# IRVLUTD/handnet-pipeline

Hardware: AMD Instinct MI355X
Metric: end-to-end frames/sec (FCOS+A2J, 640x480) (higher is better)
Workload: dtype f16x3 (fp32 values split into fp16 hi+lo, 3 MFMAs, fp32 accumulate; fp32 I/O); 1 GPU; Full HandNet pipeline (FCOS -> crop -> A2J), 640x480 RGB-D (BASELINE config 4); batch_per_gpu=32, global_batch=32, frame=640x480 RGB-D, parallelism=frames sharded over 1 GPU(s), one all-gather of per-frame records per step, rccl_ranks=1, ipc_mode=HSA_ENABLE_IPC_MODE_LEGACY=0, hipgraph=False

## Files before the change

### handnet-pipeline_amd/csrc/conv1x1_stream.hip

```cpp
#include "hn_common.h"

namespace {

typedef float f32x4 __attribute__((ext_vector_type(4)));
typedef _Float16 f16x8 __attribute__((ext_vector_type(8)));
typedef __attribute__((address_space(3))) void lds_void;

constexpr int kTileBytes = 32 * 1024;
constexpr int kStages = 2;
constexpr int kWaves = 8;
constexpr int kThreads = kWaves * 64;

struct StreamParams {
  const _Float16* x;
  const _Float16* w;
  const float* bias;
  const void* res;
  void* y;
  int M, Cout, relu, out_split, res_mode, res_split, res_h, res_w, OH, OW;
  int ys, rs;
  int tiles;
  unsigned x_records;
  unsigned mg_ohow, sh_ohow, mg_ow, sh_ow, mg_oh, sh_oh;
  int* range_flag;
};

__device__ __forceinline__ int fastdiv(int n, unsigned mg, unsigned sh) { return mg ? (int)(__umulhi((unsigned)n, mg) >> sh) : n; }

template <int CB>
__global__ __launch_bounds__(kThreads, 4) void conv1x1_stream_kernel(const StreamParams p) {
  constexpr int kTilePix = kTileBytes / (CB * 128);
  constexpr int PIX_BYTES = CB * 128;
  constexpr int CHUNKS = CB * 8;
  constexpr int TILE_BYTES = kTileBytes;
  constexpr int PASSES = TILE_BYTES / (kThreads * 16);
  static_assert(CB == 2 || CB == 4, "Cin = 64 or 128");
  static_assert(TILE_BYTES % (kThreads * 16) == 0, "a tile is a whole number of DMA passes");
  extern __shared__ __attribute__((aligned(1024))) char smem[];
  const int tid = threadIdx.x, lane = tid & 63, wave = tid >> 6, lg = lane >> 4, px = lane & 15;
  const int n0 = blockIdx.y * 256 + wave * 32;

  f16x8 bh[2][CB], bl[2][CB];
#pragma unroll
  for (int j = 0; j < 2; ++j)
#pragma unroll
    for (int cb = 0; cb < CB; ++cb) {
      const _Float16* q = p.w + ((long)(n0 + j * 16 + px) * CB + cb) * 64 + lg * 8;
      bh[j][cb] = *reinterpret_cast<const f16x8*>(q);
      bl[j][cb] = *reinterpret_cast<const f16x8*>(q + 32);
    }
  const int nsub = (lg & 1) * 16 + (lg >> 1) * 8;
  const int n = n0 + nsub;
  float* bias_lds = reinterpret_cast<float*>(smem + kStages * kTileBytes);
  if (tid < 256) bias_lds[tid] = p.bias ? p.bias[blockIdx.y * 256 + tid] : 0.f;

  const __amdgpu_buffer_rsrc_t rsrc = __builtin_amdgcn_make_buffer_rsrc((void*)p.x, 0, (int)p.x_records, 0x00020000);
  static_assert((kThreads / CHUNKS) % 16 == 0, "a DMA pass covers whole 16-pixel groups");
  const unsigned src_off = (unsigned)((tid / CHUNKS) * PIX_BYTES + (((tid % CHUNKS) ^ ((tid / CHUNKS) & 15)) << 4));
  const int wave_base = __builtin_amdgcn_readfirstlane(wave) * 64 * 16;
  auto dma_tile = [&](int t, int stage) {
#pragma unroll
    for (int ps = 0; ps < PASSES; ++ps)
      __builtin_amdgcn_raw_ptr_buffer_load_lds(rsrc, (lds_void*)(smem + stage * TILE_BYTES + ps * kThreads * 16 + wave_base), 16,
                                               (int)src_off, t * TILE_BYTES + ps * kThreads * 16, 0, 0);
  };
  auto frag = [&](int stage, int pt, int cb, int pl) {
    const int pixel = pt * 16 + px;
    return *reinterpret_cast<const f16x8*>(smem + stage * TILE_BYTES + pixel * PIX_BYTES + (((cb * 8 + pl * 4 + lg) ^ px) << 4));
  };

  const int ohow = p.OH * p.OW;
  const int t0 = blockIdx.x, dt = gridDim.x;
  dma_tile(t0, 0);
  int stage = 0;
  for (int t = t0; t < p.tiles; t += dt) {
    asm volatile("s_waitcnt vmcnt(0)" ::: "memory");
    __syncthreads();
    if (t + dt < p.tiles) dma_tile(t + dt, stage ^ 1);
#pragma unroll
    for (int pt = 0; pt < kTilePix / 16; ++pt) {
      f32x4 acc0 = {0.f, 0.f, 0.f, 0.f}, acc1 = acc0;
#pragma unroll
      for (int c2 = 0; c2 < CB; c2 += 2) {
        f16x8 ah[2], al[2];
#pragma unroll
        for (int c = 0; c < 2; ++c) {
          ah[c] = frag(stage, pt, c2 + c, 0);
          al[c] = frag(stage, pt, c2 + c, 1);
        }
#pragma unroll
        for (int c = 0; c < 2; ++c) {
          const int cb = c2 + c;
          acc0 = __builtin_amdgcn_mfma_f32_16x16x32_f16(bh[0][cb], al[c], acc0, 0, 0, 0);
          acc1 = __builtin_amdgcn_mfma_f32_16x16x32_f16(bh[1][cb], al[c], acc1, 0, 0, 0);
          acc0 = __builtin_amdgcn_mfma_f32_16x16x32_f16(bl[0][cb], ah[c], acc0, 0, 0, 0);
          acc1 = __builtin_amdgcn_mfma_f32_16x16x32_f16(bl[1][cb], ah[c], acc1, 0, 0, 0);
          acc0 = __builtin_amdgcn_mfma_f32_16x16x32_f16(bh[0][cb], ah[c], acc0, 0, 0, 0);
          acc1 = __builtin_amdgcn_mfma_f32_16x16x32_f16(bh[1][cb], ah[c], acc1, 0, 0, 0);
        }
        if (c2 + 2 < CB) __builtin_amdgcn_sched_barrier(0);
      }
#pragma unroll
      for (int r = 0; r < 4; ++r) {
        const auto s = __builtin_amdgcn_permlane16_swap(__float_as_uint(acc0[r]), __float_as_uint(acc1[r]), false, false);
        acc0[r] = __uint_as_float(s[0]);
        acc1[r] = __uint_as_float(s[1]);
      }
      const int m = t * kTilePix + pt * 16 + px;
      if (m >= p.M) continue;
      float v[8];
      const f32x4 bias0 = *reinterpret_cast<const f32x4*>(bias_lds + wave * 32 + nsub);
      const f32x4 bias1 = *reinterpret_cast<const f32x4*>(bias_lds + wave * 32 + nsub + 4);
#pragma unroll
      for (int e = 0; e < 4; ++e) {
        v[e] = acc0[e] + bias0[e];
        v[4 + e] = acc1[e] + bias1[e];
      }
      if (p.res_mode) {
        long rpix = m;
        if (p.res_mode == 2) {
          const int img = fastdiv(m, p.mg_ohow, p.sh_ohow);
          const int rem = m - img * ohow;
          const int oh = fastdiv(rem, p.mg_ow, p.sh_ow), ow = rem - oh * p.OW;
          const int sh_ = fastdiv(oh * p.res_h, p.mg_oh, p.sh_oh), sw_ = fastdiv(ow * p.res_w, p.mg_ow, p.sh_ow);
          rpix = ((long)img * p.res_h + sh_) * p.res_w + sw_;
        }
        if (p.res_split) {
          const _Float16* q16 = reinterpret_cast<const _Float16*>(p.res) + rpix * p.rs + (n >> 5) * 64 + (n & 31);
          const f16x8 rh = *reinterpret_cast<const f16x8*>(q16), rl = *reinterpret_cast<const f16x8*>(q16 + 32);
#pragma unroll
          for (int e = 0; e < 8; ++e) v[e] += (float)rh[e] + (float)rl[e];
        } else {
          const float* q32 = reinterpret_cast<const float*>(p.res) + rpix * p.rs + n;
          const f32x4 r0 = *reinterpret_cast<const f32x4*>(q32), r1 = *reinterpret_cast<const f32x4*>(q32 + 4);
#pragma unroll
          for (int e = 0; e < 4; ++e) {
            v[e] += r0[e];
            v[4 + e] += r1[e];
          }
        }
      }
      if (p.relu) {
#pragma unroll
        for (int e = 0; e < 8; ++e) v[e] = hn::relu(v[e]);
      }
      if (p.out_split) {
        if (p.range_flag) hn::range_note_n<8>(p.range_flag, v);
        f16x8 hi, lo;
#pragma unroll
        for (int e = 0; e < 8; ++e) {
          const _Float16 h = (_Float16)v[e];
          hi[e] = h;
          lo[e] = (_Float16)(v[e] - (float)h);
        }
        _Float16* q16 = reinterpret_cast<_Float16*>(p.y) + (long)m * p.ys + (n >> 5) * 64 + (n & 31);
        *reinterpret_cast<f16x8*>(q16) = hi;
        *reinterpret_cast<f16x8*>(q16 + 32) = lo;
      } else {
        float* q32 = reinterpret_cast<float*>(p.y) + (long)m * p.ys + n;
        *reinterpret_cast<f32x4*>(q32) = f32x4{v[0], v[1], v[2], v[3]};
        *reinterpret_cast<f32x4*>(q32 + 4) = f32x4{v[4], v[5], v[6], v[7]};
      }
    }
    stage ^= 1;
  }
  asm volatile("s_waitcnt vmcnt(0)" ::: "memory");
}

}

namespace hn {

static void magic_u31(unsigned d, unsigned& mg, unsigned& sh) {
  if (d <= 1) { mg = 0; sh = 0; return; }
  unsigned k = 0;
  while ((1ull << k) < d) ++k;
  mg = (unsigned)(((1ull << (31 + k)) + d - 1) / d);
  sh = k - 1;
}

bool conv1x1_stream_applies(const hn_conv_desc* d, bool has_gn, bool has_group) {
  const int64_t m = (int64_t)d->n * d->oh * d->ow;
  return !env_flags().no_stream && !has_gn && !has_group && d->r == 1 && d->s == 1 && d->stride == 1 && d->pad == 0 && d->dil == 1 &&
         (d->cin == 64 || d->cin == 128) && d->cout % 256 == 0 && d->terms != 1 && d->tile == HN_TILE_AUTO &&
         (d->in_pix_stride == 0 || d->in_pix_stride == 2 * d->cin) && (d->relu_cols == 0 || d->relu_cols >= d->cout) &&
         m >= (int64_t)65536 && (int64_t)d->oh * d->res_h < ((int64_t)1 << 31) && (int64_t)d->ow * d->res_w < ((int64_t)1 << 31) && m * d->cin * 4 < ((int64_t)1 << 31) - ((int64_t)64 << 20);
}

bool conv1x1_stream_operands_ok(const hn_conv_desc* d, const void* x16, const void* w16, const float* bias, const void* residual,
                                const void* y) {
  const int ys = d->out_pix_stride ? d->out_pix_stride : (d->out_split ? 2 : 1) * d->cout;
  const int rs = d->res_pix_stride ? d->res_pix_stride : (d->res_split ? 2 : 1) * d->cout;
  return (uintptr_t)x16 % 16 == 0 && (uintptr_t)w16 % 16 == 0 && (uintptr_t)y % 16 == 0 && (!bias || (uintptr_t)bias % 16 == 0) &&
         (!residual || (uintptr_t)residual % 16 == 0) && (d->out_split ? ys % 64 == 0 : ys % 4 == 0) &&
         (d->res_mode == 0 || (d->res_split ? rs % 64 == 0 : rs % 4 == 0));
}

int conv1x1_stream(const hn_conv_desc* d, const void* x16, const void* w16, const float* bias, const void* residual, void* y,
                   hipStream_t st) {
  StreamParams p;
  p.x = (const _Float16*)x16; p.w = (const _Float16*)w16; p.bias = bias; p.res = d->res_mode ? residual : nullptr; p.y = y;
  p.M = d->n * d->oh * d->ow; p.Cout = d->cout; p.relu = d->relu_cols > 0; p.out_split = d->out_split;
  p.res_mode = d->res_mode; p.res_split = d->res_split; p.res_h = d->res_h; p.res_w = d->res_w; p.OH = d->oh; p.OW = d->ow;
  p.ys = d->out_pix_stride ? d->out_pix_stride : (d->out_split ? 2 : 1) * d->cout;
  p.rs = d->res_pix_stride ? d->res_pix_stride : (d->res_split ? 2 : 1) * d->cout;
  const int tile_pix = kTileBytes / (d->cin * 4);
  p.tiles = cdiv(p.M, tile_pix);
  magic_u31((unsigned)(d->oh * d->ow), p.mg_ohow, p.sh_ohow);
  magic_u31((unsigned)d->ow, p.mg_ow, p.sh_ow);
  magic_u31((unsigned)d->oh, p.mg_oh, p.sh_oh);
  p.x_records = (unsigned)((int64_t)p.M * d->cin * 4);
  p.range_flag = range_flag_ptr();
  const int cb = d->cin / 32;
  const int lds = kStages * kTileBytes + 1024;
  int dev = 0, cus = 256;
  HN_CHECK_HIP(hipGetDevice(&dev));
  static int cu_count[64] = {};
  if (dev >= 0 && dev < 64) {
    if (!cu_count[dev]) {
      hipDeviceProp_t prop;
      HN_CHECK_HIP(hipGetDeviceProperties(&prop, dev));
      cu_count[dev] = prop.multiProcessorCount;
    }
    cus = cu_count[dev];
  }
  const int groups = d->cout / 256;
  int gx = cus * 2 / groups;
  gx = gx < 1 ? 1 : (gx > p.tiles ? p.tiles : gx);
  static bool attr_set[2][64] = {};
  auto set_attr = [&](const void* fn, int which) -> int {
    if (dev < 0 || dev >= 64 || !attr_set[which][dev]) {
      HN_CHECK_HIP(hipFuncSetAttribute(fn, hipFuncAttributeMaxDynamicSharedMemorySize, lds));
      if (dev >= 0 && dev < 64) attr_set[which][dev] = true;
    }
    return HN_OK;
  };
  if (cb == 2) {
    const int s = set_attr((const void*)conv1x1_stream_kernel<2>, 0);
    if (s != HN_OK) return s;
    hipLaunchKernelGGL(conv1x1_stream_kernel<2>, dim3(gx, groups), dim3(kThreads), lds, st, p);
  } else {
    const int s = set_attr((const void*)conv1x1_stream_kernel<4>, 1);
    if (s != HN_OK) return s;
    hipLaunchKernelGGL(conv1x1_stream_kernel<4>, dim3(gx, groups), dim3(kThreads), lds, st, p);
  }
  HN_CHECK_LAUNCH("conv1x1_stream_kernel");
  return HN_OK;
}

}
```

### handnet-pipeline_amd/csrc/hn_common.h

```cpp
#pragma once
#include <hip/hip_runtime.h>
#include <stdarg.h>
#include <stdint.h>
#include <stdio.h>

#include "../../include/handnet_hip.h"

namespace hn {

char* err_buf();
int fail(int code, const char* fmt, ...);
int* range_flag_ptr();
struct EnvFlags {
  bool no_rs, no_rs32, split_generic, no_halo, no_thin, thin_tap, thin_flat, no_fuse_last_gn, pre_generic, no_multi,
      halo_stamps, splitk_fill512, no_stream, no_mixed, no_deepk, no_fused_reduce, thin_nogroup;
};
const EnvFlags& env_flags();
struct Tuning {
  double splitk_fix = 1.0, splitk_tk = 1.0, splitk_red0 = 1.0, splitk_plane = 1.0;
};
const Tuning& tuning();
bool conv3x3_halo_applies(const hn_conv_desc* d, bool has_gn, bool has_group, const void* residual);
bool conv3x3_halo_operands_ok(const hn_conv_desc* d, const void* x16, const void* w16, const float* bias, const void* residual,
                              const void* y);
int conv3x3_halo(const hn_conv_desc* d, const void* x16, const void* w16, const float* bias, const void* residual, void* y,
                 hipStream_t st);
int stem_pool_direct(const void* x16, int n, int ph, int pw, const void* w16, const float* bias, void* y, int terms, hipStream_t st);
bool conv1x1_stream_applies(const hn_conv_desc* d, bool has_gn, bool has_group);
bool conv1x1_stream_operands_ok(const hn_conv_desc* d, const void* x16, const void* w16, const float* bias, const void* residual,
                                const void* y);
int conv1x1_stream(const hn_conv_desc* d, const void* x16, const void* w16, const float* bias, const void* residual, void* y,
                   hipStream_t st);

struct CarryHook {
  const void* job;
  bool dry;
};
int launch_conv_carry(const void* conv_params, size_t conv_params_bytes, int grid_x, int groups, int terms, int lds_bytes,
                      const void* job, hipStream_t st);
int conv_grouped_run(const hn_conv_desc* d, const hn_conv_group* group, void* stream, const CarryHook* carry);

int tickets_nonzero_main(int64_t* count);
int tickets_nonzero_multi(int64_t* count);

#define HN_CHECK_ARG(cond, ...)                          \
  do {                                                   \
    if (!(cond)) return hn::fail(HN_ERR_ARG, __VA_ARGS__); \
  } while (0)

#define HN_CHECK_HIP(expr)                                                         \
  do {                                                                             \
    hipError_t e_ = (expr);                                                        \
    if (e_ != hipSuccess)                                                          \
      return hn::fail(HN_ERR_HIP, "%s failed: %s", #expr, hipGetErrorString(e_)); \
  } while (0)

#define HN_CHECK_LAUNCH(name)                                                          \
  do {                                                                                 \
    hipError_t e_ = hipGetLastError();                                                 \
    if (e_ != hipSuccess)                                                              \
      return hn::fail(HN_ERR_HIP, "launch of %s failed: %s", name, hipGetErrorString(e_)); \
  } while (0)

static inline int cdiv(int64_t a, int64_t b) { return (int)((a + b - 1) / b); }

__device__ __forceinline__ void range_note(int* flag, float v) {
  if (!(fabsf(v) <= 65504.f)) *flag = 1;
}
__device__ __forceinline__ float max_nan(float a, float b) { return __builtin_elementwise_maximum(a, b); }
__device__ __forceinline__ float relu(float v) { return max_nan(v, 0.f); }
__device__ __forceinline__ float range_mag(float a, float b) { return max_nan(fabsf(a), fabsf(b)); }
__device__ __forceinline__ bool range_bad(float v) { return !(fabsf(v) <= 65504.f); }
template <int N>
__device__ __forceinline__ void range_note_n(int* flag, const float (&v)[N]) {
  float m = fabsf(v[0]);
#pragma unroll
  for (int e = 1; e < N; ++e) m = max_nan(m, fabsf(v[e]));
  if (!(m <= 65504.f)) *flag = 1;
}
__device__ __forceinline__ void range_note_input(int* flag, float v) {
  if (!(fabsf(v) <= 65504.f)) flag[fabsf(v) <= 3.402823466e38f ? 1 : 2] = 1;
}

}
```

### handnet-pipeline_amd/csrc/hn_common.hip

```cpp
#include "hn_common.h"

#include <stdlib.h>

#include <string.h>

__device__ int g_range_flag[4];
static thread_local int g_range_check_on = 0;
static thread_local int* g_range_bound = nullptr;
struct RangeScope { int on; int* bound; };
static thread_local RangeScope g_range_stack[8];
static thread_local int g_range_depth = 0;

namespace hn {

int* range_flag_ptr() {
  if (!g_range_check_on) return nullptr;
  if (g_range_bound) return g_range_bound;
  static int* ptrs[64] = {nullptr};
  int dev = 0;
  if (hipGetDevice(&dev) != hipSuccess || dev < 0 || dev >= 64) return nullptr;
  if (!ptrs[dev]) {
    void* p = nullptr;
    if (hipGetSymbolAddress(&p, HIP_SYMBOL(g_range_flag)) != hipSuccess) return nullptr;
    ptrs[dev] = (int*)p;
  }
  return ptrs[dev];
}

char* err_buf() {
  static thread_local char buf[512] = {0};
  return buf;
}

int fail(int code, const char* fmt, ...) {
  va_list ap;
  va_start(ap, fmt);
  vsnprintf(err_buf(), 512, fmt, ap);
  va_end(ap);
  return code;
}

}

extern "C" int hn_abi_version(void) { return HN_ABI_VERSION; }

extern "C" int hn_debug_tickets_nonzero(int64_t* count) {
  HN_CHECK_ARG(count, "hn_debug_tickets_nonzero: null pointer");
  *count = 0;
  if (int rc = hn::tickets_nonzero_main(count)) return rc;
  return hn::tickets_nonzero_multi(count);
}

namespace hn {
static EnvFlags g_env = {};
const EnvFlags& env_flags() { return g_env; }
static Tuning g_tuning;
const Tuning& tuning() { return g_tuning; }
}

extern "C" int hn_set_tuning(const char* name, double value) {
  HN_CHECK_ARG(name && value > 0.0, "hn_set_tuning: null name or non-positive value");
  struct Entry { const char* name; double hn::Tuning::*field; };
  static const Entry table[] = {{"splitk_fix", &hn::Tuning::splitk_fix}, {"splitk_tk", &hn::Tuning::splitk_tk},
                                {"splitk_red0", &hn::Tuning::splitk_red0}, {"splitk_plane", &hn::Tuning::splitk_plane}};
  for (const Entry& e : table)
    if (strcmp(e.name, name) == 0) {
      hn::g_tuning.*(e.field) = value;
      return HN_OK;
    }
  return hn::fail(HN_ERR_ARG, "hn_set_tuning: unknown constant '%s'", name);
}

extern "C" int hn_set_form(const char* name, int value) {
  HN_CHECK_ARG(name, "hn_set_form: null name");
  struct Entry { const char* name; bool hn::EnvFlags::*field; };
  static const Entry table[] = {
      {"conv_no_rs", &hn::EnvFlags::no_rs},
      {"conv_no_rs32", &hn::EnvFlags::no_rs32},
      {"split_generic", &hn::EnvFlags::split_generic},
      {"conv_no_halo", &hn::EnvFlags::no_halo},
      {"preprocess_generic", &hn::EnvFlags::pre_generic},
      {"conv_no_multi", &hn::EnvFlags::no_multi},
      {"no_fuse_last_gn", &hn::EnvFlags::no_fuse_last_gn},
      {"no_thin_outputs", &hn::EnvFlags::no_thin},
      {"thin_form_tap", &hn::EnvFlags::thin_tap},
      {"thin_form_flat", &hn::EnvFlags::thin_flat},
      {"thin_no_group", &hn::EnvFlags::thin_nogroup},
      {"halo_stamps", &hn::EnvFlags::halo_stamps},
      {"splitk_fill512", &hn::EnvFlags::splitk_fill512},
      {"conv_no_stream", &hn::EnvFlags::no_stream},
      {"conv_no_mixed", &hn::EnvFlags::no_mixed},
      {"conv_no_deepk", &hn::EnvFlags::no_deepk},
      {"conv_no_fused_reduce", &hn::EnvFlags::no_fused_reduce},
  };
  for (const Entry& e : table)
    if (strcmp(e.name, name) == 0) {
      hn::g_env.*(e.field) = value != 0;
      return HN_OK;
    }
  return hn::fail(HN_ERR_ARG, "hn_set_form: unknown form '%s'", name);
}

extern "C" const char* hn_last_error(void) { return hn::err_buf(); }

extern "C" int hn_device_info(int* cu_count, int* clock_khz, char* arch_name, int arch_name_len) {
  int dev = 0;
  HN_CHECK_HIP(hipGetDevice(&dev));
  hipDeviceProp_t prop;
  HN_CHECK_HIP(hipGetDeviceProperties(&prop, dev));
  if (cu_count) *cu_count = prop.multiProcessorCount;
  if (clock_khz) *clock_khz = prop.clockRate;
  if (arch_name && arch_name_len > 0) {
    strncpy(arch_name, prop.gcnArchName, arch_name_len - 1);
    arch_name[arch_name_len - 1] = 0;
  }
  return HN_OK;
}

extern "C" int hn_device_pci_bus_id(char* out, int out_len) {
  HN_CHECK_ARG(out && out_len >= 16, "hn_device_pci_bus_id: buffer of at least 16 bytes");
  int dev = 0;
  HN_CHECK_HIP(hipGetDevice(&dev));
  HN_CHECK_HIP(hipDeviceGetPCIBusId(out, out_len, dev));
  return HN_OK;
}

extern "C" int hn_event_create(void** ev) {
  HN_CHECK_ARG(ev, "hn_event_create: null");
  hipEvent_t e;
  HN_CHECK_HIP(hipEventCreate(&e));
  *ev = (void*)e;
  return HN_OK;
}

extern "C" int hn_event_destroy(void* ev) {
  HN_CHECK_HIP(hipEventDestroy((hipEvent_t)ev));
  return HN_OK;
}

extern "C" int hn_event_record(void* ev, void* stream) {
  HN_CHECK_HIP(hipEventRecord((hipEvent_t)ev, (hipStream_t)stream));
  return HN_OK;
}

extern "C" int hn_event_elapsed_ms(void* start, void* stop, float* ms) {
  HN_CHECK_ARG(ms, "hn_event_elapsed_ms: null");
  HN_CHECK_HIP(hipEventSynchronize((hipEvent_t)stop));
  HN_CHECK_HIP(hipEventElapsedTime(ms, (hipEvent_t)start, (hipEvent_t)stop));
  return HN_OK;
}

extern "C" int hn_range_check_enable(int on) {
  g_range_check_on = on ? 1 : 0;
  return HN_OK;
}

extern "C" int hn_range_check_enabled(void) { return g_range_check_on; }

extern "C" int hn_range_check_bind(int32_t* block) {
  g_range_bound = block;
  return HN_OK;
}

extern "C" int hn_range_scope_begin(int32_t* block, int on) {
  HN_CHECK_ARG(g_range_depth < 8, "hn_range_scope_begin: more than 8 nested scopes on this thread");
  g_range_stack[g_range_depth++] = RangeScope{g_range_check_on, g_range_bound};
  g_range_check_on = on ? 1 : 0;
  g_range_bound = on ? block : nullptr;
  return HN_OK;
}

extern "C" int hn_range_scope_end(void) {
  HN_CHECK_ARG(g_range_depth > 0, "hn_range_scope_end: no open scope on this thread");
  const RangeScope s = g_range_stack[--g_range_depth];
  g_range_check_on = s.on;
  g_range_bound = s.bound;
  return HN_OK;
}

extern "C" int hn_range_check_fetch(int* flag, int reset, void* stream) {
  HN_CHECK_ARG(flag, "hn_range_check_fetch: null");
  void* p = nullptr;
  int words[4] = {0, 0, 0, 0};
  HN_CHECK_HIP(hipGetSymbolAddress(&p, HIP_SYMBOL(g_range_flag)));
  HN_CHECK_HIP(hipMemcpyAsync(words, p, sizeof(words), hipMemcpyDeviceToHost, (hipStream_t)stream));
  HN_CHECK_HIP(hipStreamSynchronize((hipStream_t)stream));
  *flag = (words[0] ? HN_RANGE_ACTIVATION : 0) | (words[1] ? HN_RANGE_INPUT : 0) | (words[2] ? HN_RANGE_INPUT_NONFINITE : 0);
  if (reset) {
    HN_CHECK_HIP(hipMemsetAsync(p, 0, sizeof(words), (hipStream_t)stream));
    HN_CHECK_HIP(hipStreamSynchronize((hipStream_t)stream));
  }
  return HN_OK;
}

namespace {
__global__ void range_collect_kernel(int* __restrict__ flags, int* __restrict__ dst) {
  const int t = threadIdx.x;
  if (t < 4) {
    dst[t] = flags[t];
    flags[t] = 0;
  }
}
}

extern "C" int hn_range_check_collect(int32_t* block, int32_t* dst, void* stream) {
  HN_CHECK_ARG(dst, "hn_range_check_collect: null");
  void* p = block;
  if (!p) HN_CHECK_HIP(hipGetSymbolAddress(&p, HIP_SYMBOL(g_range_flag)));
  hipLaunchKernelGGL(range_collect_kernel, dim3(1), dim3(64), 0, (hipStream_t)stream, (int*)p, dst);
  HN_CHECK_LAUNCH("range_collect_kernel");
  return HN_OK;
}

namespace {
__global__ __launch_bounds__(64) void clock_sample_kernel(unsigned long long ticks, float* mhz) {
  const unsigned long long r0 = __builtin_amdgcn_s_memrealtime();
  const unsigned long long c0 = __builtin_amdgcn_s_memtime();
  unsigned long long r1 = r0;
  for (long guard = 0; guard < (1L << 26) && r1 - r0 < ticks; ++guard) {
    __builtin_amdgcn_s_sleep(64);
    r1 = __builtin_amdgcn_s_memrealtime();
  }
  const unsigned long long c1 = __builtin_amdgcn_s_memtime();
  if (threadIdx.x == 0) mhz[0] = (float)((double)(c1 - c0) / ((double)(r1 - r0) * 0.01));
}
}

extern "C" int hn_clock_sample(int micros, float* mhz, void* stream) {
  HN_CHECK_ARG(mhz, "hn_clock_sample: null");
  HN_CHECK_ARG(micros > 0 && micros <= 2000000, "hn_clock_sample: micros must be in 1..2e6");
  hipLaunchKernelGGL(clock_sample_kernel, dim3(1), dim3(64), 0, (hipStream_t)stream, (unsigned long long)micros * 100ull, mhz);
  HN_CHECK_LAUNCH("clock_sample_kernel");
  return HN_OK;
}
```

### handnet-pipeline_amd/hn_amd/forms.py

```python
from __future__ import annotations

import os

ENGINE_DEFAULTS = dict(
    head_streams=1,
    group_convs=True,
    fuse_stem_pool=True,
    fuse_last_gn=True,
    thin_outputs=True,
    conv_multi=True,
    conv_multi_fcos=True,
    tower_carry=True,
)
ACTIVE = dict(ENGINE_DEFAULTS)

_LIB_ENV = {
    "HN_CONV_NO_RS": ("conv_no_rs", None), "HN_CONV_NO_RS32": ("conv_no_rs32", None),
    "HN_SPLIT_GENERIC": ("split_generic", None),
    "HN_CONV_NO_HALO": ("conv_no_halo", None), "HN_PREPROCESS_GENERIC": ("preprocess_generic", None),
    "HN_CONV_NO_MULTI": ("conv_no_multi", None), "HN_HALO_STAMPS": ("halo_stamps", None),
    "HN_SPLITK_FILL512": ("splitk_fill512", None), "HN_CONV_NO_STREAM": ("conv_no_stream", None),
    "HN_CONV_NO_MIXED": ("conv_no_mixed", None), "HN_CONV_NO_DEEPK": ("conv_no_deepk", None),
    "HN_CONV_NO_FUSED_REDUCE": ("conv_no_fused_reduce", None), "HN_THIN_NO_GROUP": ("thin_no_group", None),
}


def engine_forms(overrides=None) -> dict:
    f = dict(ACTIVE)
    if overrides:
        unknown = set(overrides) - set(ENGINE_DEFAULTS)
        if unknown:
            raise KeyError(f"unknown engine forms: {sorted(unknown)}")
        f.update(overrides)
    return f


def apply_env(environ=None) -> dict:
    from . import ops
    env = os.environ if environ is None else environ
    done = {}
    for var, (form, _) in _LIB_ENV.items():
        if var in env:
            ops.set_form(form, True)
            done[var] = form
    if env.get("HN_FUSE_LAST_GN") == "0":
        ops.set_form("no_fuse_last_gn", True)
        ACTIVE["fuse_last_gn"] = False
        done["HN_FUSE_LAST_GN"] = "0"
    if env.get("HN_THIN_OUTPUTS") == "0":
        ops.set_form("no_thin_outputs", True)
        ACTIVE["thin_outputs"] = False
        done["HN_THIN_OUTPUTS"] = "0"
    if env.get("HN_THIN_FORM", "")[:1] in ("t", "f"):
        ops.set_form("thin_form_tap" if env["HN_THIN_FORM"][0] == "t" else "thin_form_flat", True)
        done["HN_THIN_FORM"] = env["HN_THIN_FORM"]
    for var, key in (("HN_GROUP_CONVS", "group_convs"), ("HN_FUSE_STEM_POOL", "fuse_stem_pool"), ("HN_CONV_MULTI", "conv_multi"),
                     ("HN_CONV_MULTI_FCOS", "conv_multi_fcos"), ("HN_TOWER_CARRY", "tower_carry")):
        if var in env:
            ACTIVE[key] = env[var] != "0"
            done[var] = env[var]
    if "HN_CONV_MULTI" in env and "HN_CONV_MULTI_FCOS" not in env:
        ACTIVE["conv_multi_fcos"] = ACTIVE["conv_multi"]
    if "HN_HEAD_STREAMS" in env:
        ACTIVE["head_streams"] = int(env["HN_HEAD_STREAMS"])
        done["HN_HEAD_STREAMS"] = env["HN_HEAD_STREAMS"]
    if "HN_SPLITK" in env:
        ops.SPLITK = env["HN_SPLITK"] != "0"
        done["HN_SPLITK"] = env["HN_SPLITK"]
    if "HN_SPLITK_EAGER" in env:
        ops.SPLITK_EAGER = env["HN_SPLITK_EAGER"] == "1"
        done["HN_SPLITK_EAGER"] = env["HN_SPLITK_EAGER"]
    for var in env:
        if var.startswith("HN_TUNE_"):
            from . import _lib
            ops.check(_lib.load().hn_set_tuning(var[8:].lower().encode(), float(env[var])), "hn_set_tuning")
            done[var] = env[var]
    if "HN_CANDIDATES_CHUNKED" in env:
        ops.CANDIDATES_CHUNKED = env["HN_CANDIDATES_CHUNKED"] != "0"
        done["HN_CANDIDATES_CHUNKED"] = env["HN_CANDIDATES_CHUNKED"]
    return done
```

Measured before the change: 1189 frames/s.

## Extend streaming 1x1 conv kernel to Cin 256/512 and retune dispatch thresholds

```diff
diff --git a/handnet-pipeline_amd/csrc/conv1x1_stream.hip b/handnet-pipeline_amd/csrc/conv1x1_stream.hip
--- a/handnet-pipeline_amd/csrc/conv1x1_stream.hip
+++ b/handnet-pipeline_amd/csrc/conv1x1_stream.hip
@@ -27,42 +27,53 @@
 
 __device__ __forceinline__ int fastdiv(int n, unsigned mg, unsigned sh) { return mg ? (int)(__umulhi((unsigned)n, mg) >> sh) : n; }
 
-template <int CB>
-__global__ __launch_bounds__(kThreads, 4) void conv1x1_stream_kernel(const StreamParams p) {
+template <int CB, int NJ>
+__global__ __launch_bounds__(kThreads, CB * NJ >= 16 ? 2 : 4) void conv1x1_stream_kernel(const StreamParams p) {
   constexpr int kTilePix = kTileBytes / (CB * 128);
   constexpr int PIX_BYTES = CB * 128;
   constexpr int CHUNKS = CB * 8;
   constexpr int TILE_BYTES = kTileBytes;
   constexpr int PASSES = TILE_BYTES / (kThreads * 16);
-  static_assert(CB == 2 || CB == 4, "Cin = 64 or 128");
+  typedef _Float16 f16xv __attribute__((ext_vector_type(4 * NJ)));
+  constexpr int GW = 128 * NJ;
+  constexpr int NV = 4 * NJ;
+  static_assert(((CB == 2 || CB == 4) && NJ == 2) || CB == 8 || (CB == 16 && NJ == 1), "Cin 64 / 128 (256 columns), 256, 512 (128)");
+  static_assert(kTilePix % 16 == 0 && CHUNKS >= 16, "whole 16-pixel groups; the XOR stays inside a pixel's row");
   static_assert(TILE_BYTES % (kThreads * 16) == 0, "a tile is a whole number of DMA passes");
   extern __shared__ __attribute__((aligned(1024))) char smem[];
   const int tid = threadIdx.x, lane = tid & 63, wave = tid >> 6, lg = lane >> 4, px = lane & 15;
-  const int n0 = blockIdx.y * 256 + wave * 32;
-
-  f16x8 bh[2][CB], bl[2][CB];
-#pragma unroll
-  for (int j = 0; j < 2; ++j)
+  const int n0 = blockIdx.y * GW + wave * 16 * NJ;
+
+  f16x8 bh[NJ][CB], bl[NJ][CB];
+#pragma unroll
+  for (int j = 0; j < NJ; ++j)
 #pragma unroll
     for (int cb = 0; cb < CB; ++cb) {
       const _Float16* q = p.w + ((long)(n0 + j * 16 + px) * CB + cb) * 64 + lg * 8;
       bh[j][cb] = *reinterpret_cast<const f16x8*>(q);
       bl[j][cb] = *reinterpret_cast<const f16x8*>(q + 32);
     }
-  const int nsub = (lg & 1) * 16 + (lg >> 1) * 8;
+  const int nsub = NJ == 2 ? (lg & 1) * 16 + (lg >> 1) * 8 : lg * 4;
   const int n = n0 + nsub;
   float* bias_lds = reinterpret_cast<float*>(smem + kStages * kTileBytes);
-  if (tid < 256) bias_lds[tid] = p.bias ? p.bias[blockIdx.y * 256 + tid] : 0.f;
+  if (tid < GW) bias_lds[tid] = p.bias ? p.bias[blockIdx.y * GW + tid] : 0.f;
 
   const __amdgpu_buffer_rsrc_t rsrc = __builtin_amdgcn_make_buffer_rsrc((void*)p.x, 0, (int)p.x_records, 0x00020000);
-  static_assert((kThreads / CHUNKS) % 16 == 0, "a DMA pass covers whole 16-pixel groups");
+  constexpr int PASS_PIX = kThreads / CHUNKS;
+  constexpr bool kOneOffset = PASS_PIX % 16 == 0;
   const unsigned src_off = (unsigned)((tid / CHUNKS) * PIX_BYTES + (((tid % CHUNKS) ^ ((tid / CHUNKS) & 15)) << 4));
   const int wave_base = __builtin_amdgcn_readfirstlane(wave) * 64 * 16;
   auto dma_tile = [&](int t, int stage) {
 #pragma unroll
-    for (int ps = 0; ps < PASSES; ++ps)
+    for (int ps = 0; ps < PASSES; ++ps) {
+      unsigned off = src_off;
+      if constexpr (!kOneOffset) {
+        const int pix = ps * PASS_PIX + tid / CHUNKS;
+        off = (unsigned)((tid / CHUNKS) * PIX_BYTES + (((tid % CHUNKS) ^ (pix & 15)) << 4));
+      }
       __builtin_amdgcn_raw_ptr_buffer_load_lds(rsrc, (lds_void*)(smem + stage * TILE_BYTES + ps * kThreads * 16 + wave_base), 16,
-                                               (int)src_off, t * TILE_BYTES + ps * kThreads * 16, 0, 0);
+                                               (int)off, t * TILE_BYTES + ps * kThreads * 16, 0, 0);
+    }
   };
   auto frag = [&](int stage, int pt, int cb, int pl) {
     const int pixel = pt * 16 + px;
@@ -92,29 +103,32 @@
         for (int c = 0; c < 2; ++c) {
           const int cb = c2 + c;
           acc0 = __builtin_amdgcn_mfma_f32_16x16x32_f16(bh[0][cb], al[c], acc0, 0, 0, 0);
-          acc1 = __builtin_amdgcn_mfma_f32_16x16x32_f16(bh[1][cb], al[c], acc1, 0, 0, 0);
+          if constexpr (NJ == 2) acc1 = __builtin_amdgcn_mfma_f32_16x16x32_f16(bh[NJ - 1][cb], al[c], acc1, 0, 0, 0);
           acc0 = __builtin_amdgcn_mfma_f32_16x16x32_f16(bl[0][cb], ah[c], acc0, 0, 0, 0);
-          acc1 = __builtin_amdgcn_mfma_f32_16x16x32_f16(bl[1][cb], ah[c], acc1, 0, 0, 0);
+          if constexpr (NJ == 2) acc1 = __builtin_amdgcn_mfma_f32_16x16x32_f16(bl[NJ - 1][cb], ah[c], acc1, 0, 0, 0);
           acc0 = __builtin_amdgcn_mfma_f32_16x16x32_f16(bh[0][cb], ah[c], acc0, 0, 0, 0);
-          acc1 = __builtin_amdgcn_mfma_f32_16x16x32_f16(bh[1][cb], ah[c], acc1, 0, 0, 0);
+          if constexpr (NJ == 2) acc1 = __builtin_amdgcn_mfma_f32_16x16x32_f16(bh[NJ - 1][cb], ah[c], acc1, 0, 0, 0);
         }
         if (c2 + 2 < CB) __builtin_amdgcn_sched_barrier(0);
       }
-#pragma unroll
-      for (int r = 0; r < 4; ++r) {
-        const auto s = __builtin_amdgcn_permlane16_swap(__float_as_uint(acc0[r]), __float_as_uint(acc1[r]), false, false);
-        acc0[r] = __uint_as_float(s[0]);
-        acc1[r] = __uint_as_float(s[1]);
+      if constexpr (NJ == 2) {
+#pragma unroll
+        for (int r = 0; r < 4; ++r) {
+          const auto s = __builtin_amdgcn_permlane16_swap(__float_as_uint(acc0[r]), __float_as_uint(acc1[r]), false, false);
+          acc0[r] = __uint_as_float(s[0]);
+          acc1[r] = __uint_as_float(s[1]);
+        }
       }
       const int m = t * kTilePix + pt * 16 + px;
       if (m >= p.M) continue;
-      float v[8];
-      const f32x4 bias0 = *reinterpret_cast<const f32x4*>(bias_lds + wave * 32 + nsub);
-      const f32x4 bias1 = *reinterpret_cast<const f32x4*>(bias_lds + wave * 32 + nsub + 4);
-#pragma unroll
-      for (int e = 0; e < 4; ++e) {
-        v[e] = acc0[e] + bias0[e];
-        v[4 + e] = acc1[e] + bias1[e];
+      float v[NV];
+      const f32x4 bias0 = *reinterpret_cast<const f32x4*>(bias_lds + wave * 16 * NJ + nsub);
+#pragma unroll
+      for (int e = 0; e < 4; ++e) v[e] = acc0[e] + bias0[e];
+      if constexpr (NJ == 2) {
+        const f32x4 bias1 = *reinterpret_cast<const f32x4*>(bias_lds + wave * 16 * NJ + nsub + 4);
+#pragma unroll
+        for (int e = 0; e < 4; ++e) v[4 + e] = acc1[e] + bias1[e];
       }
       if (p.res_mode) {
         long rpix = m;
@@ -127,39 +141,41 @@
         }
         if (p.res_split) {
           const _Float16* q16 = reinterpret_cast<const _Float16*>(p.res) + rpix * p.rs + (n >> 5) * 64 + (n & 31);
-          const f16x8 rh = *reinterpret_cast<const f16x8*>(q16), rl = *reinterpret_cast<const f16x8*>(q16 + 32);
-#pragma unroll
-          for (int e = 0; e < 8; ++e) v[e] += (float)rh[e] + (float)rl[e];
+          const f16xv rh = *reinterpret_cast<const f16xv*>(q16), rl = *reinterpret_cast<const f16xv*>(q16 + 32);
+#pragma unroll
+          for (int e = 0; e < NV; ++e) v[e] += (float)rh[e] + (float)rl[e];
         } else {
           const float* q32 = reinterpret_cast<const float*>(p.res) + rpix * p.rs + n;
-          const f32x4 r0 = *reinterpret_cast<const f32x4*>(q32), r1 = *reinterpret_cast<const f32x4*>(q32 + 4);
-#pragma unroll
-          for (int e = 0; e < 4; ++e) {
-            v[e] += r0[e];
-            v[4 + e] += r1[e];
+          const f32x4 r0 = *reinterpret_cast<const f32x4*>(q32);
+#pragma unroll
+          for (int e = 0; e < 4; ++e) v[e] += r0[e];
+          if constexpr (NJ == 2) {
+            const f32x4 r1 = *reinterpret_cast<const f32x4*>(q32 + 4);
+#pragma unroll
+            for (int e = 0; e < 4; ++e) v[4 + e] += r1[e];
           }
         }
       }
       if (p.relu) {
 #pragma unroll
-        for (int e = 0; e < 8; ++e) v[e] = hn::relu(v[e]);
+        for (int e = 0; e < NV; ++e) v[e] = hn::relu(v[e]);
       }
       if (p.out_split) {
-        if (p.range_flag) hn::range_note_n<8>(p.range_flag, v);
-        f16x8 hi, lo;
-#pragma unroll
-        for (int e = 0; e < 8; ++e) {
+        if (p.range_flag) hn::range_note_n<NV>(p.range_flag, v);
+        f16xv hi, lo;
+#pragma unroll
+        for (int e = 0; e < NV; ++e) {
           const _Float16 h = (_Float16)v[e];
           hi[e] = h;
           lo[e] = (_Float16)(v[e] - (float)h);
         }
         _Float16* q16 = reinterpret_cast<_Float16*>(p.y) + (long)m * p.ys + (n >> 5) * 64 + (n & 31);
-        *reinterpret_cast<f16x8*>(q16) = hi;
-        *reinterpret_cast<f16x8*>(q16 + 32) = lo;
+        *reinterpret_cast<f16xv*>(q16) = hi;
+        *reinterpret_cast<f16xv*>(q16 + 32) = lo;
       } else {
         float* q32 = reinterpret_cast<float*>(p.y) + (long)m * p.ys + n;
         *reinterpret_cast<f32x4*>(q32) = f32x4{v[0], v[1], v[2], v[3]};
-        *reinterpret_cast<f32x4*>(q32 + 4) = f32x4{v[4], v[5], v[6], v[7]};
+        if constexpr (NJ == 2) *reinterpret_cast<f32x4*>(q32 + 4) = f32x4{v[4], v[5], v[6], v[7]};
       }
     }
     stage ^= 1;
@@ -179,12 +195,25 @@
   sh = k - 1;
 }
 
+static int stream_tile_pix(int cin) { return kTileBytes / (cin * 4); }
+static bool stream_big_group(const hn_conv_desc* d) { return d->cin == 256 && d->cout % 256 == 0; }
+
 bool conv1x1_stream_applies(const hn_conv_desc* d, bool has_gn, bool has_group) {
+  const EnvFlags& ef = env_flags();
   const int64_t m = (int64_t)d->n * d->oh * d->ow;
-  return !env_flags().no_stream && !has_gn && !has_group && d->r == 1 && d->s == 1 && d->stride == 1 && d->pad == 0 && d->dil == 1 &&
-         (d->cin == 64 || d->cin == 128) && d->cout % 256 == 0 && d->terms != 1 && d->tile == HN_TILE_AUTO &&
-         (d->in_pix_stride == 0 || d->in_pix_stride == 2 * d->cin) && (d->relu_cols == 0 || d->relu_cols >= d->cout) &&
-         m >= (int64_t)65536 && (int64_t)d->oh * d->res_h < ((int64_t)1 << 31) && (int64_t)d->ow * d->res_w < ((int64_t)1 << 31) && m * d->cin * 4 < ((int64_t)1 << 31) - ((int64_t)64 << 20);
+  if (ef.no_stream || has_gn || has_group || d->r != 1 || d->s != 1 || d->stride != 1 || d->pad != 0 || d->dil != 1 || d->terms == 1 ||
+      d->tile != HN_TILE_AUTO || !(d->in_pix_stride == 0 || d->in_pix_stride == 2 * d->cin) ||
+      !(d->relu_cols == 0 || d->relu_cols >= d->cout) || m < 1 || (int64_t)d->oh * d->res_h >= ((int64_t)1 << 31) ||
+      (int64_t)d->ow * d->res_w >= ((int64_t)1 << 31) || m * d->cin * 4 >= ((int64_t)1 << 31) - ((int64_t)64 << 20))
+    return false;
+  if (d->cin == 64 || d->cin == 128) {
+    if (d->cout % 256) return false;
+    if (ef.stream_narrow) return m >= 65536;
+    return ef.stream_force || (m + stream_tile_pix(d->cin) - 1) / stream_tile_pix(d->cin) * (d->cout / 256) >= (d->cin == 64 ? 240 : 800);
+  }
+  if (ef.stream_narrow || d->cout % 128) return false;
+  if (d->cin == 256) return ef.stream_force || (m >= (stream_big_group(d) ? 49152 : 90112) && m <= 262144);
+  return d->cin == 512 && ef.stream_force;
 }
 
 bool conv1x1_stream_operands_ok(const hn_conv_desc* d, const void* x16, const void* w16, const float* bias, const void* residual,
@@ -204,14 +233,13 @@
   p.res_mode = d->res_mode; p.res_split = d->res_split; p.res_h = d->res_h; p.res_w = d->res_w; p.OH = d->oh; p.OW = d->ow;
   p.ys = d->out_pix_stride ? d->out_pix_stride : (d->out_split ? 2 : 1) * d->cout;
   p.rs = d->res_pix_stride ? d->res_pix_stride : (d->res_split ? 2 : 1) * d->cout;
-  const int tile_pix = kTileBytes / (d->cin * 4);
-  p.tiles = cdiv(p.M, tile_pix);
+  const int cb = d->cin / 32;
+  p.tiles = cdiv(p.M, stream_tile_pix(d->cin));
   magic_u31((unsigned)(d->oh * d->ow), p.mg_ohow, p.sh_ohow);
   magic_u31((unsigned)d->ow, p.mg_ow, p.sh_ow);
   magic_u31((unsigned)d->oh, p.mg_oh, p.sh_oh);
   p.x_records = (unsigned)((int64_t)p.M * d->cin * 4);
   p.range_flag = range_flag_ptr();
-  const int cb = d->cin / 32;
   const int lds = kStages * kTileBytes + 1024;
   int dev = 0, cus = 256;
   HN_CHECK_HIP(hipGetDevice(&dev));
@@ -224,26 +252,28 @@
     }
     cus = cu_count[dev];
   }
-  const int groups = d->cout / 256;
-  int gx = cus * 2 / groups;
+  const bool big_group = stream_big_group(d);
+  const int groups = d->cout / (cb >= 8 && !big_group ? 128 : 256);
+  int gx = (int)(cus * (cb >= 16 || big_group ? 1 : 2) / groups * tuning().stream_grid);
   gx = gx < 1 ? 1 : (gx > p.tiles ? p.tiles : gx);
-  static bool attr_set[2][64] = {};
-  auto set_attr = [&](const void* fn, int which) -> int {
+  static bool attr_set[5][64] = {};
+  auto launch = [&](auto kernel, int which) -> int {
     if (dev < 0 || dev >= 64 || !attr_set[which][dev]) {
-      HN_CHECK_HIP(hipFuncSetAttribute(fn, hipFuncAttributeMaxDynamicSharedMemorySize, lds));
+      HN_CHECK_HIP(hipFuncSetAttribute((const void*)kernel, hipFuncAttributeMaxDynamicSharedMemorySize, lds));
       if (dev >= 0 && dev < 64) attr_set[which][dev] = true;
     }
+    hipLaunchKernelGGL(kernel, dim3(gx, groups), dim3(kThreads), lds, st, p);
     return HN_OK;
   };
-  if (cb == 2) {
-    const int s = set_attr((const void*)conv1x1_stream_kernel<2>, 0);
-    if (s != HN_OK) return s;
-    hipLaunchKernelGGL(conv1x1_stream_kernel<2>, dim3(gx, groups), dim3(kThreads), lds, st, p);
-  } else {
-    const int s = set_attr((const void*)conv1x1_stream_kernel<4>, 1);
-    if (s != HN_OK) return s;
-    hipLaunchKernelGGL(conv1x1_stream_kernel<4>, dim3(gx, groups), dim3(kThreads), lds, st, p);
-  }
+  int s = HN_OK;
+  switch (cb) {
+    case 2: s = launch(conv1x1_stream_kernel<2, 2>, 0); break;
+    case 4: s = launch(conv1x1_stream_kernel<4, 2>, 1); break;
+    case 8: s = big_group ? launch(conv1x1_stream_kernel<8, 2>, 4) : launch(conv1x1_stream_kernel<8, 1>, 2); break;
+    case 16: s = launch(conv1x1_stream_kernel<16, 1>, 3); break;
+    default: return fail(HN_ERR_ARG, "conv1x1_stream: no kernel for Cin = %d", d->cin);
+  }
+  if (s != HN_OK) return s;
   HN_CHECK_LAUNCH("conv1x1_stream_kernel");
   return HN_OK;
 }
diff --git a/handnet-pipeline_amd/csrc/hn_common.h b/handnet-pipeline_amd/csrc/hn_common.h
--- a/handnet-pipeline_amd/csrc/hn_common.h
+++ b/handnet-pipeline_amd/csrc/hn_common.h
@@ -13,11 +13,11 @@
 int* range_flag_ptr();
 struct EnvFlags {
   bool no_rs, no_rs32, split_generic, no_halo, no_thin, thin_tap, thin_flat, no_fuse_last_gn, pre_generic, no_multi,
-      halo_stamps, splitk_fill512, no_stream, no_mixed, no_deepk, no_fused_reduce, thin_nogroup;
+      halo_stamps, splitk_fill512, no_stream, no_mixed, no_deepk, no_fused_reduce, thin_nogroup, stream_narrow, stream_force;
 };
 const EnvFlags& env_flags();
 struct Tuning {
-  double splitk_fix = 1.0, splitk_tk = 1.0, splitk_red0 = 1.0, splitk_plane = 1.0;
+  double splitk_fix = 1.0, splitk_tk = 1.0, splitk_red0 = 1.0, splitk_plane = 1.0, stream_grid = 1.0;
 };
 const Tuning& tuning();
 bool conv3x3_halo_applies(const hn_conv_desc* d, bool has_gn, bool has_group, const void* residual);
diff --git a/handnet-pipeline_amd/csrc/hn_common.hip b/handnet-pipeline_amd/csrc/hn_common.hip
--- a/handnet-pipeline_amd/csrc/hn_common.hip
+++ b/handnet-pipeline_amd/csrc/hn_common.hip
@@ -62,7 +62,8 @@
   HN_CHECK_ARG(name && value > 0.0, "hn_set_tuning: null name or non-positive value");
   struct Entry { const char* name; double hn::Tuning::*field; };
   static const Entry table[] = {{"splitk_fix", &hn::Tuning::splitk_fix}, {"splitk_tk", &hn::Tuning::splitk_tk},
-                                {"splitk_red0", &hn::Tuning::splitk_red0}, {"splitk_plane", &hn::Tuning::splitk_plane}};
+                                {"splitk_red0", &hn::Tuning::splitk_red0}, {"splitk_plane", &hn::Tuning::splitk_plane},
+                                {"stream_grid", &hn::Tuning::stream_grid}};
   for (const Entry& e : table)
     if (strcmp(e.name, name) == 0) {
       hn::g_tuning.*(e.field) = value;
@@ -89,6 +90,8 @@
       {"halo_stamps", &hn::EnvFlags::halo_stamps},
       {"splitk_fill512", &hn::EnvFlags::splitk_fill512},
       {"conv_no_stream", &hn::EnvFlags::no_stream},
+      {"conv_stream_narrow", &hn::EnvFlags::stream_narrow},
+      {"conv_stream_force", &hn::EnvFlags::stream_force},
       {"conv_no_mixed", &hn::EnvFlags::no_mixed},
       {"conv_no_deepk", &hn::EnvFlags::no_deepk},
       {"conv_no_fused_reduce", &hn::EnvFlags::no_fused_reduce},
diff --git a/handnet-pipeline_amd/hn_amd/forms.py b/handnet-pipeline_amd/hn_amd/forms.py
--- a/handnet-pipeline_amd/hn_amd/forms.py
+++ b/handnet-pipeline_amd/hn_amd/forms.py
@@ -51,6 +51,9 @@
         ops.set_form("no_thin_outputs", True)
         ACTIVE["thin_outputs"] = False
         done["HN_THIN_OUTPUTS"] = "0"
+    if env.get("HN_STREAM_WIDE") == "0":
+        ops.set_form("conv_stream_narrow", True)
+        done["HN_STREAM_WIDE"] = "0"
     if env.get("HN_THIN_FORM", "")[:1] in ("t", "f"):
         ops.set_form("thin_form_tap" if env["HN_THIN_FORM"][0] == "t" else "thin_form_flat", True)
         done["HN_THIN_FORM"] = env["HN_THIN_FORM"]
```

Result: no change. 1193 frames/s, median of 6 (+0.3%).
